# FrancisTheCat/raytracing_c

Measured on AMD Instinct MI355X. Metric: Mray/s, higher is better.
Workload: dtype f32; 1 GPU; helmet.glb 1920x1080, 256 spp, 8 bounces (BASELINE.json configs[2]); partition=single GPU

## Files before the change

### raytracing_c_amd/csrc/rt_dev.hip.h

```cpp
#ifndef RT_DEV_HIP_H
#define RT_DEV_HIP_H

#include <hip/hip_runtime.h>
#include <stdint.h>

#include "rt_device.h"
#include "../../include/rt_math.h"

#ifndef RT_SCALAR_TEX
#define RT_SCALAR_TEX 1
#endif
#ifndef RT_SCALAR_MATS
#define RT_SCALAR_MATS 1
#endif
#ifndef RT_LEAF_PAIRS
#define RT_LEAF_PAIRS 0
#endif

#define RT_BLOCK_WAVES 4
#define RT_BLOCK_THREADS (RT_BLOCK_WAVES * 64)

#define CNT_PATHS 0
#define CNT_RAYS 1
#define CNT_NODES 2
// ... 807 lines not shown
  } else {
    t = normalize_dev(rt_v3_cross(normal, rt_v3_make(1, 0, 0)));
  }
  b = rt_v3_cross(normal, t);

  BrdfIn bi;
  bi.roughness = roughness;
  bi.metalness = metalness;
  bi.base_color = base_color;
  bi.sheen = m2.y;
  bi.sheen_tint = m2.z;
  bi.aniso2 = m2.w * m2.w;

  rt_v3 neg = rt_v3_scale(in.direction, -1.0f);
  rt_v3 in_dir = rt_v3_make(rt_v3_dot(t, neg), rt_v3_dot(b, neg), rt_v3_dot(normal, neg));
  rt_v3 o, rgb;
  float a;
  sample_disney(bi, in_dir, rng, o, rgb, a);

  out_dir = rt_v3_comb3(t, o.x, b, o.y, normal, o.z);
  if (a > 0.0f) {
    tint = rt_v3_make(rgb.x / a, rgb.y / a, rgb.z / a);
  } else {
    terminate = true;
  }
}

template <class PT>
__device__ __forceinline__ void primary_ray(const PT &P, int x, int y, int sample, rt_v3 &o, rt_v3 &d) {
  float inv_width = P.inv_width;
  float inv_height = P.inv_height;
  float aspect = P.aspect;
  float jitter = rt_hash12((float)x * 50.0f + (float)sample, (float)y);
  float uvx = rt_madd(((float)x + jitter - 0.5f) * 2.0f, inv_width, -1.0f);
  float uvy = rt_madd(((float)y + jitter - 0.5f) * 2.0f, inv_height, -1.0f);
  float dx = uvx * aspect, dy = -uvy, dz = -P.focal_length;
  float inv_length = rcp_exact(rt_sqrtf(rt_dot3(dx, dx, dy, dy, dz, dz)));
  float rx = rt_dot3(P.cam[0][0], dx, P.cam[0][1], dy, P.cam[0][2], dz);
  float ry = rt_dot3(P.cam[1][0], dx, P.cam[1][1], dy, P.cam[1][2], dz);
  float rz = rt_dot3(P.cam[2][0], dx, P.cam[2][1], dy, P.cam[2][2], dz);
  o = rt_v3_make(P.cam[0][3], P.cam[1][3], P.cam[2][3]);
  d = rt_v3_make(rx * inv_length, ry * inv_length, rz * inv_length);
}

template <bool SHORT_DIV = false>
__device__ __forceinline__ void ray_setup(Ray3 &r, rt_v3 o, rt_v3 d) {
  r.o = o;
  r.d = d;
  if (SHORT_DIV) {
    r.inv_x = rcp_exact(d.x);
    r.inv_y = rcp_exact(d.y);
    r.inv_z = rcp_exact(d.z);
  } else {
    r.inv_x = 1.0f / d.x;
    r.inv_y = 1.0f / d.y;
    r.inv_z = 1.0f / d.z;
  }
  r.fast = rt_slab_fast(o.x, o.y, o.z, r.inv_x, r.inv_y, r.inv_z, rt_slab_bias(o.x, r.inv_x), rt_slab_bias(o.y, r.inv_y), rt_slab_bias(o.z, r.inv_z));
}

template <class PT>
__device__ __forceinline__ bool shade_hit(const PT &P, const HitRec &hit, rt_v3 &org, rt_v3 &dir,
                                          rt_v3 &tint, rt_v3 &emis, uint32_t &rng, int &bounce,
                                          LaneCounters &cn, rt_v3 &radiance) {
  bool done = false;
  const float *tb = P.tris + (size_t)hit.tri * 28;
  float4 q0 = ld4(tb, 0), q1 = ld4(tb, 1), q2 = ld4(tb, 2), q3 = ld4(tb, 3);
  float4 q4 = ld4(tb, 4), q5 = ld4(tb, 5), q6 = ld4(tb, 6);
  float t1 = hit.u, t2 = hit.v;
  float t0 = 1.0f - t1 - t2;
  rt_v3 point = rt_v3_madd(dir, hit.t, org);
  rt_v3 n_geo = rt_v3_make(q0.x, q0.y, q0.z);
  rt_v3 n_int = rt_v3_make(rt_dot3(q1.x, t0, q2.x, t1, q3.x, t2),
                           rt_dot3(q1.y, t0, q2.y, t1, q3.y, t2),
                           rt_dot3(q1.z, t0, q2.z, t1, q3.z, t2));
  if (rt_v3_dot(n_geo, dir) > 0.0f || rt_v3_dot(n_int, dir) > 0.0f) {
    org = rt_v3_madd(dir, RT_EPS, point);
  } else {
    ShadeIn in;
    in.direction = dir;
    in.normal = normalize_dev(n_int);
    in.tangent = rt_v3_make(q4.x, q4.y, q4.z);
    in.bitangent = rt_v3_make(q5.x, q5.y, q5.z);
    in.uvx = rt_dot3(q1.w, t0, q3.w, t1, q5.w, t2);
    in.uvy = rt_dot3(q2.w, t0, q4.w, t1, q6.x, t2);
    rt_v3 out_dir, s_tint, s_emis;
    bool terminate;
    cn.shades += 1;
    shade(P, as_i(q0.w), in, rng, out_dir, s_tint, s_emis, terminate, cn);
    emis = rt_v3_mul_add(s_emis, tint, emis);
    if (terminate) {
      done = true;
      radiance = emis;
    } else {
      dir = out_dir;
      tint = rt_v3_mul(tint, s_tint);
      float below = (rt_v3_dot(n_geo, out_dir) < 0.0f) ? 1.0f : 0.0f;
      float bias = (0.5f - below) * 2.0f * RT_EPS;
      org = rt_v3_madd(n_geo, bias, point);
    }
  }
  if (!done) {
    bounce += 1;
    if (bounce >= P.max_bounces) {
      done = true;
      radiance = emis;
    }
  }
  return done;
}

#define PH_NEED 0
#define PH_POP  1
#define PH_NODE 2
#define PH_LEAF 3
#define PH_HIT  4
#define PH_MISS 5

#define RT_PARK_FIELDS 18
#define RT_PARK_CAP 128
static_assert(RT_PARK_FIELDS * RT_PARK_CAP == RT_PARK_RECORD_DWORDS, "park slice size (rt_device.h) out of step");
#ifndef RT_PARK_DENSE
#define RT_PARK_DENSE 48
#endif
#ifndef RT_JOIN_CHOICES
#define RT_JOIN_CHOICES 4
#endif
#ifndef RT_PYR_NUM
#define RT_PYR_NUM 3
#define RT_PYR_DEN 4
#define RT_PYR_MIN 8
#endif
#define RT_STEAL_TRIES  16
#ifndef RT_LEAF_TRIP
#define RT_LEAF_TRIP 1
#endif
#ifndef RT_LEAF_CULL_MAX
#define RT_LEAF_CULL_MAX 4
#endif
#ifndef RT_PARK_STOP_PATHS
#define RT_PARK_STOP_PATHS 0
#endif

__device__ __forceinline__ float *lds_at(float4 *smem, int byte_off) {
  asm volatile("" : "+s"(byte_off));
  return reinterpret_cast<float *>(reinterpret_cast<char *>(smem) + byte_off);
}
__device__ __forceinline__ int lane_now() {
  unsigned ones = ~0u;
  asm volatile("" : "+s"(ones));
  return (int)__builtin_amdgcn_mbcnt_hi(ones, __builtin_amdgcn_mbcnt_lo(ones, 0u));
}

__device__ __forceinline__ uint32_t pyramid_cull_mask(const float4 *lds_nodes, const float *pyr, int node) {
  const int lane = lane_now();
  const float *nb = reinterpret_cast<const float *>(lds_nodes + lds_node_f4(node)) + (lane & 7);
  const float *pl = pyr + ((lane >> 3) & 3) * 4;
  const float ox = pyr[16], oy = pyr[17], oz = pyr[18];
  const float mnx = nb[0], mny = nb[8], mnz = nb[16], mxx = nb[24], mxy = nb[32], mxz = nb[40];
  const float nx = pl[0], ny = pl[1], nz = pl[2];
  const bool empty = mnx == 0.0f && mny == 0.0f && mnz == 0.0f && mxx == 0.0f && mxy == 0.0f && mxz == 0.0f;
  const float lox = nx * (mnx - ox), hix = nx * (mxx - ox), loy = ny * (mny - oy), hiy = ny * (mxy - oy);
  const float loz = nz * (mnz - oz), hiz = nz * (mxz - oz);
  const float nearest = fminf(lox, hix) + fminf(loy, hiy) + fminf(loz, hiz);
  const float extent = fmaxf(fabsf(lox), fabsf(hix)) + fmaxf(fabsf(loy), fabsf(hiy)) + fmaxf(fabsf(loz), fabsf(hiz));
  const float coarse = fabsf(nx) * (fabsf(ox) + fmaxf(fabsf(mnx), fabsf(mxx))) + fabsf(ny) * (fabsf(oy) + fmaxf(fabsf(mny), fabsf(mxy))) +
                       fabsf(nz) * (fabsf(oz) + fmaxf(fabsf(mnz), fabsf(mxz)));
  const bool outside = empty || nearest > 1e-3f * extent + 1e-6f * coarse;
  const uint32_t m = (uint32_t)__ballot(outside);
  return (m | (m >> 8) | (m >> 16) | (m >> 24)) & 0xFFu;
}

__device__ __forceinline__ float slab_entry_ordered(const Ray3 &r, const rt_v3 &bs, const char *nbase, int k, int nx, int ny, int nz, float t_max) {
  const char *b = nbase + k * 4;
  const float sx = rt_slab_t_fast(*reinterpret_cast<const float *>(b + nx), r.o.x, r.inv_x, bs.x);
  const float bx = rt_slab_t_fast(*reinterpret_cast<const float *>(b + (96 - nx)), r.o.x, r.inv_x, bs.x);
  const float sy = rt_slab_t_fast(*reinterpret_cast<const float *>(b + 32 + ny), r.o.y, r.inv_y, bs.y);
  const float by = rt_slab_t_fast(*reinterpret_cast<const float *>(b + 32 + (96 - ny)), r.o.y, r.inv_y, bs.y);
  const float sz = rt_slab_t_fast(*reinterpret_cast<const float *>(b + 64 + nz), r.o.z, r.inv_z, bs.z);
  const float bz = rt_slab_t_fast(*reinterpret_cast<const float *>(b + 64 + (96 - nz)), r.o.z, r.inv_z, bs.z);
  const float t_minv = fmax_hw(RT_EPS, fmax_hw(sx, fmax_hw(sy, sz)));
  const float t_maxv = fmin_hw(t_max, fmin_hw(bx, fmin_hw(by, bz)));
  return (t_minv < t_maxv) ? t_minv : RT_INF;
}

__device__ __forceinline__ uint32_t node_enter_few(const Ray3 &r, const float4 *lds_nodes, int node, uint32_t surv,
                                                   float hit_t) {
  const char *nbase = reinterpret_cast<const char *>(lds_nodes + lds_node_f4(node));
  const int nx = (as_i(r.inv_x) >> 31) & 96, ny = (as_i(r.inv_y) >> 31) & 96, nz = (as_i(r.inv_z) >> 31) & 96;
  const rt_v3 bs = slab_bias3(r);
  const int n = (int)__popc(surv);
  const int k0 = (int)__builtin_ctz(surv);
  const int e0 = as_i(slab_entry_ordered(r, bs, nbase, k0, nx, ny, nz, hit_t));
  const uint32_t f0 = 1u - (((uint32_t)e0 + 0x00800000u) >> 31);
  LGM("nfew_ret1");
  if (n == 1) return (uint32_t)k0 | (f0 << 24);
  surv &= surv - 1u;
  const int k1 = (int)__builtin_ctz(surv);
  const int e1 = as_i(slab_entry_ordered(r, bs, nbase, k1, nx, ny, nz, hit_t));
  const uint32_t f1 = 1u - (((uint32_t)e1 + 0x00800000u) >> 31);
  LGM("nfew_two");
  if (n == 2) {
    const bool swap = e1 < e0;
    const uint32_t first = swap ? (uint32_t)k1 : (uint32_t)k0, second = swap ? (uint32_t)k0 : (uint32_t)k1;
    return first | (second << 3) | ((f0 + f1) << 24);
  }
  LGM("nfew_ret2");
  surv &= surv - 1u;
  const int k2 = (int)__builtin_ctz(surv);
  const int e2 = as_i(slab_entry_ordered(r, bs, nbase, k2, nx, ny, nz, hit_t));
  const uint32_t f2 = 1u - (((uint32_t)e2 + 0x00800000u) >> 31);
  int e3 = 0x7F800000, k3 = 0;
  uint32_t f3 = 0;
  LGM("nfew_four_begin");
  if (n == 4) {
    surv &= surv - 1u;
    k3 = (int)__builtin_ctz(surv);
      e3 = as_i(slab_entry_ordered(r, bs, nbase, k3, nx, ny, nz, hit_t));
    f3 = 1u - (((uint32_t)e3 + 0x00800000u) >> 31);
  }
  LGM("nfew_four_end");
  const int e[4] = {e0, e1, e2, e3};
  const int kk[4] = {k0, k1, k2, k3};
  int rank[4] = {0, 1, 2, 3};
#pragma unroll
  for (int j = 0; j < 4; j++) {
#pragma unroll
    for (int k = j + 1; k < 4; k++) {
      int kb = (int)((uint32_t)(e[k] - e[j]) >> 31);
      rank[j] += kb;
      rank[k] -= kb;
    }
  }
  uint32_t w = 0;
#pragma unroll
  for (int j = 0; j < 4; j++) w |= (uint32_t)kk[j] << (3 * rank[j]);
  return w | ((f0 + f1 + f2 + f3) << 24);
}

__device__ __forceinline__ uint32_t pyramid_cull_tris(const float *leaves, const float *pyr, int g) {
  const int lane = lane_now();
  const float *tb = leaves + (size_t)g * 72 + (lane & 7);
  const float *pl = pyr + ((lane >> 3) & 3) * 4;
  const float ox = pyr[16], oy = pyr[17], oz = pyr[18];
  const float nx = pl[0], ny = pl[1], nz = pl[2];
  const float ax = tb[0], e1x = tb[8], e2x = tb[16], ay = tb[24], e1y = tb[32], e2y = tb[40], az = tb[48], e1z = tb[56], e2z = tb[64];
  bool outside = true;
#pragma unroll
  for (int v = 0; v < 3; v++) {
    const float vx = v == 0 ? ax : (v == 1 ? ax + e1x : ax + e2x);
    const float vy = v == 0 ? ay : (v == 1 ? ay + e1y : ay + e2y);
    const float vz = v == 0 ? az : (v == 1 ? az + e1z : az + e2z);
    const float px = nx * (vx - ox), py = ny * (vy - oy), pz = nz * (vz - oz);
    const float val = px + py + pz;
    const float extent = fabsf(px) + fabsf(py) + fabsf(pz);
    const float coarse = fabsf(nx) * (fabsf(ox) + fabsf(vx)) + fabsf(ny) * (fabsf(oy) + fabsf(vy)) + fabsf(nz) * (fabsf(oz) + fabsf(vz));
    outside = outside && (val > 1e-3f * extent + 1e-6f * coarse);
  }
  const uint32_t m = (uint32_t)__ballot(outside);
  return (m | (m >> 8) | (m >> 16) | (m >> 24)) & 0xFFu;
}

template <bool SHORT_DIV>
__device__ __forceinline__ void tri_test_uniform(const Ray3 &r, rt_v3 a, rt_v3 edge1, rt_v3 edge2, int k, float &best, float &bu, float &bv, int &bi) {
  rt_v3 rxe2 = rt_v3_cross(r.d, edge2);
  float det = rt_v3_dot(edge1, rxe2);
  float inv_det = SHORT_DIV ? rcp_leaf(det) : 1.0f / det;
  rt_v3 s = rt_v3_sub(r.o, a);
  rt_v3 sxe1 = rt_v3_cross(s, edge1);
  float u = inv_det * rt_v3_dot(s, rxe2);
  float v = inv_det * rt_v3_dot(r.d, sxe1);
  float t = inv_det * rt_v3_dot(edge2, sxe1);
  bool miss = (u < -RT_EPS) || (u > 1.0f + RT_EPS) || (v < -RT_EPS) || (u + v > 1.0f + RT_EPS) || (t < RT_EPS);
  if (SHORT_DIV) {
    if (!miss && t < best) { best = t; bi = k; bu = u; bv = v; }
  } else {
    float dist = miss ? RT_INF : t;
    dist = (dist > 0.0f) ? dist : RT_INF;
    if (dist < best) { best = dist; bi = k; bu = u; bv = v; }
  }
}
template <bool SHORT_DIV>
__device__ __forceinline__ bool leaf_test_uniform(const RT_KParams &P, const Ray3 &r, int g, uint32_t surv, HitRec &hit) {
  float best = RT_INF, bu = 0.0f, bv = 0.0f;
  int   bi = 0;
  cfloat *lb = as_scalar_ptr(P.leaves) + (size_t)g * 72;
  while (surv) {
    const int k0 = (int)__builtin_ctz(surv);
    surv &= surv - 1u;
#if RT_LEAF_TRIP == 1
    {
      cfloat *t0 = lb + k0;
      tri_test_uniform<SHORT_DIV>(r, rt_v3_make(t0[0], t0[24], t0[48]), rt_v3_make(t0[8], t0[32], t0[56]), rt_v3_make(t0[16], t0[40], t0[64]),
                                  k0, best, bu, bv, bi);
      continue;
    }
#endif
    const bool two = surv != 0u;
    const int k1 = two ? (int)__builtin_ctz(surv) : k0;
    surv &= surv - 1u;
    cfloat *t0 = lb + k0, *t1 = lb + k1;
    const rt_v3 a0 = rt_v3_make(t0[0], t0[24], t0[48]), e10 = rt_v3_make(t0[8], t0[32], t0[56]), e20 = rt_v3_make(t0[16], t0[40], t0[64]);
    const rt_v3 a1 = rt_v3_make(t1[0], t1[24], t1[48]), e11 = rt_v3_make(t1[8], t1[32], t1[56]), e21 = rt_v3_make(t1[16], t1[40], t1[64]);
    tri_test_uniform<SHORT_DIV>(r, a0, e10, e20, k0, best, bu, bv, bi);
    if (two) tri_test_uniform<SHORT_DIV>(r, a1, e11, e21, k1, best, bu, bv, bi);
  }
// ... 288 lines not shown
```

### raytracing_c_amd/csrc/rt_kernels.hip

```cpp

#include "rt_dev.hip.h"


#ifdef RT_LEDGER
#define RT_LEDGER_WAVES 8192
__device__ uint32_t g_ledger[RT_LEDGER_WAVES * RT_LEDGER_ROW];
__global__ void rt_ledger_reduce_kernel(unsigned long long *counters) {
  const int slot = threadIdx.x;
  if (slot >= LG_N || slot >= RT_LEDGER_ROW) return;
  unsigned long long sum = 0ull;
  for (int w = 0; w < RT_LEDGER_WAVES; w++) sum += g_ledger[w * RT_LEDGER_ROW + slot];
  counters[8 + slot] = sum;
}
#endif

typedef const RT_KView __attribute__((address_space(4))) *RT_KViewP;
template <bool VIEWS> struct CamSrc { typedef RT_KArgs type; };
template <> struct CamSrc<true> { typedef RT_KViewP type; };

template <int WAVES, bool LDSN, int MIN_WAVES_PER_SIMD, bool SHORT_DIV, bool VIEWS>
__global__ __launch_bounds__(WAVES * 64, MIN_WAVES_PER_SIMD) void rt_path_kernel_stream(RT_KParams P) {
  extern __shared__ float4 smem[];
  const int lane = threadIdx.x & 63;
  const int wave = threadIdx.x >> 6;
// ... 69 lines not shown
      RT_KArgs A = cold_args();
      const int n_tiles = A->n_tiles;
      const uint32_t *open_groups = A->open_groups, *tile_next = A->tile_next;
      const int n_groups = (n_tiles + 63) >> 6;
      const int g_rounds = (n_groups + 63) >> 6;
      const uint32_t hsh = ((uint32_t)wave_id * 2654435761u + (uint32_t)steal_tries * 40503u) >> 8;
      const int g_start = (int)(hsh % (uint32_t)g_rounds);
      for (int i = 0; i < g_rounds && tile_idx < 0; i++) {
        int r = g_start + i;
        if (r >= g_rounds) r -= g_rounds;
        int g = r * 64 + lane;
        uint32_t n_open = 0;
        if (g < n_groups) n_open = __hip_atomic_load(&open_groups[g], __ATOMIC_RELAXED, __HIP_MEMORY_SCOPE_AGENT);
        unsigned long long gm = __ballot(n_open != 0u);
        while (gm && tile_idx < 0) {
          int nth = (int)((hsh >> 6) % (uint32_t)__popcll(gm));
          unsigned long long m = gm;
          for (int k = 0; k < nth; k++) m &= m - 1ull;
          int gl = (int)__builtin_ctzll(m);
          gm &= ~(1ull << gl);
          int cand = (r * 64 + gl) * 64 + lane;
          uint32_t taken = 0xFFFFFFFFu;
          if (cand < n_tiles) taken = __hip_atomic_load(&tile_next[cand], __ATOMIC_RELAXED, __HIP_MEMORY_SCOPE_AGENT);
          unsigned long long open = __ballot(taken < n_chunks_tile);
          if (open) {
            const int n_open_tiles = (int)__popcll(open);
            int best = 0;
            uint32_t best_taken = 0xFFFFFFFFu;
#pragma unroll
            for (int c = 0; c < RT_JOIN_CHOICES; c++) {
              int nt = (int)(((hsh >> 12) * (uint32_t)(2 * c + 1) + (uint32_t)c * 7u) % (uint32_t)n_open_tiles);
              unsigned long long mm = open;
              for (int k = 0; k < nt; k++) mm &= mm - 1ull;
              const int pk_lane = (int)__builtin_ctzll(mm);
              const uint32_t tk = (uint32_t)__builtin_amdgcn_readlane((int)taken, pk_lane);
              if (tk < best_taken) { best_taken = tk; best = pk_lane; }
            }
            tile_idx = cand - lane + best;
          }
        }
      }
      LGT1(LG_CYC_JOIN);
      if (tile_idx < 0) break;
    }

    int tile_x0, tile_y0;
    RT_KViewP vrec = nullptr;
    {
      RT_KArgs A = cold_args();
      int vt = tile_idx;
      if constexpr (VIEWS) {
        const int tu = __builtin_amdgcn_readfirstlane(tile_idx);
        const uint32_t view = (uint32_t)tu / (uint32_t)A->tiles_per_view;
        vt = tu - (int)view * A->tiles_per_view;
        vrec = (RT_KViewP)A->views + view;
      }
      const int lchunk = vt >> 4, sub = vt & 15;
      const int chunk = A->local_chunks[lchunk];
      const int chunks_x = A->chunks_x;
      tile_x0 = (chunk % chunks_x) * 32 + (sub & 3) * 8;
      tile_y0 = (chunk / chunks_x) * 32 + (sub >> 2) * 8;
      if (tile_x0 >= A->width || tile_y0 >= A->height) {
        if (lane == 0) {
          uint32_t old = atomicMax(&A->tile_next[tile_idx], n_chunks_tile);
          if (old < n_chunks_tile) atomicSub(&A->open_groups[tile_idx >> 6], 1u);
        }
        continue;
      }
    }
    bool tile_root_miss = false;
    if (leaf_level >= 0) {
      RT_KArgs A = cold_args();
      typename CamSrc<VIEWS>::type S;
      if constexpr (VIEWS) S = vrec; else S = A;
      const float m = 0.05f;
      const float ux0 = ((float)tile_x0 - 0.5f - m) * 2.0f * A->inv_width - 1.0f;
      const float ux1 = ((float)tile_x0 + 7.5f + m) * 2.0f * A->inv_width - 1.0f;
      const float uy0 = ((float)tile_y0 - 0.5f - m) * 2.0f * A->inv_height - 1.0f;
      const float uy1 = ((float)tile_y0 + 7.5f + m) * 2.0f * A->inv_height - 1.0f;
      const float asp = A->aspect, fl = S->focal_length;
      rt_v3 c[4];
#pragma unroll
      for (int q = 0; q < 4; q++) {
        float cx = ((q == 1 || q == 2) ? ux1 : ux0) * asp, cy = -((q >= 2) ? uy1 : uy0), cz = -fl;
        c[q] = rt_v3_make(S->cam[0][0] * cx + S->cam[0][1] * cy + S->cam[0][2] * cz,
                          S->cam[1][0] * cx + S->cam[1][1] * cy + S->cam[1][2] * cz,
                          S->cam[2][0] * cx + S->cam[2][1] * cy + S->cam[2][2] * cz);
      }
      const rt_v3 o = rt_v3_make(S->cam[0][3], S->cam[1][3], S->cam[2][3]);
      rt_v3 pn[4];
#pragma unroll
      for (int q = 0; q < 4; q++) {
        rt_v3 n = rt_v3_cross(c[q], c[(q + 1) & 3]);
        if (rt_v3_dot(n, c[(q + 2) & 3]) > 0.0f) n = rt_v3_scale(n, -1.0f);
        pn[q] = n;
      }
      float *pyr = lds_at(smem, pyr_off);
      if (lane == 0) {
#pragma unroll
        for (int q = 0; q < 4; q++) { pyr[q * 4 + 0] = pn[q].x; pyr[q * 4 + 1] = pn[q].y; pyr[q * 4 + 2] = pn[q].z; }
        pyr[16] = o.x; pyr[17] = o.y; pyr[18] = o.z;
      }
      if (lane < 40) reinterpret_cast<uint32_t *>(pyr)[24 + lane] = 0u;
      bool may_hit = false;
      if (lane < 8) {
        const float *nb = P.nodes + lane;
        rt_v3 lo = rt_v3_make(nb[0] - o.x, nb[8] - o.y, nb[16] - o.z);
        rt_v3 hi = rt_v3_make(nb[24] - o.x, nb[32] - o.y, nb[40] - o.z);
        const bool empty = nb[0] == 0.0f && nb[8] == 0.0f && nb[16] == 0.0f && nb[24] == 0.0f && nb[32] == 0.0f && nb[40] == 0.0f;
        bool outside = empty;
#pragma unroll
        for (int q = 0; q < 4; q++) {
          rt_v3 n = pn[q];
          float lox = n.x * lo.x, hix = n.x * hi.x, loy = n.y * lo.y, hiy = n.y * hi.y, loz = n.z * lo.z, hiz = n.z * hi.z;
          float nearest = fminf(lox, hix) + fminf(loy, hiy) + fminf(loz, hiz);
          float extent = fmaxf(fabsf(lox), fabsf(hix)) + fmaxf(fabsf(loy), fabsf(hiy)) + fmaxf(fabsf(loz), fabsf(hiz));
          float coarse = fabsf(n.x) * (fabsf(o.x) + fmaxf(fabsf(nb[0]), fabsf(nb[24]))) + fabsf(n.y) * (fabsf(o.y) + fmaxf(fabsf(nb[8]), fabsf(nb[32]))) +
                         fabsf(n.z) * (fabsf(o.z) + fmaxf(fabsf(nb[16]), fabsf(nb[40])));
          if (nearest > 1e-3f * extent + 1e-6f * coarse) outside = true;
        }
        may_hit = !outside;
      }
      tile_root_miss = __ballot(may_hit) == 0ull;
    }
    const uint32_t rays_before = w_rays;
    LG(LG_TILE_X, 1);
    LGM("tile_end");
    LGT1(LG_CYC_TILE);

    int   phase = PH_NEED;
    int   pix = 0, bounce = 0;
    uint32_t rng = 0;
    Ray3  ray;
    ray_setup(ray, rt_v3_make(0, 0, 0), rt_v3_make(0, 0, 1));
    rt_v3 tint = rt_v3_make(1, 1, 1), emis = rt_v3_make(0, 0, 0);
    int   level = -1, node = 0, child = 0;
    uint32_t cur = 0, dirty = 0, live = 0;
    HitRec hit;
    hit.t = RT_INF; hit.tri = -1; hit.u = 0; hit.v = 0;

    bool tile_open = true;
    int  c_next = 0, c_end = 0, c_x0 = 0, c_y = 0, c_pix0 = 0, c_s0 = 0;
    uint32_t u_cur = 0, u_end = 0, grab = queue_open ? (uint32_t)cold_args()->grab_max : 1u;
    bool took_any = false;
    int  n_parked = 0;
    uint32_t *park = cold_args()->park;

#ifndef RT_NO_SKY_LOOP
    if (tile_root_miss && cold_args()->max_bounces > 0) {
      RT_KArgs A = cold_args();
      typename CamSrc<VIEWS>::type S;
      if constexpr (VIEWS) S = vrec; else S = A;
      const int width = A->width, height = A->height, sample_first = A->sample_first, sample_end = A->sample_end;
      const uint32_t n_sb = (uint32_t)A->n_sample_blocks, gmax = (uint32_t)A->grab_max;
      PrimaryParams PP;
#pragma unroll
      for (int i = 0; i < 3; i++)
#pragma unroll
        for (int j = 0; j < 4; j++) PP.cam[i][j] = S->cam[i][j];
      PP.focal_length = S->focal_length; PP.inv_width = A->inv_width; PP.inv_height = A->inv_height; PP.aspect = A->aspect;
      ShadeParamsLds SP;
      SP.tris = nullptr; SP.mats = nullptr; SP.textures = A->textures; SP.texels = A->texels;
      SP.bg_texture = A->bg_texture; SP.max_bounces = A->max_bounces;
      uint32_t *tile_next = A->tile_next, *open_groups = A->open_groups;
      uint32_t n_sky = 0;
      for (;;) {
        if (c_next >= c_end) {
          if (u_cur + 1u < u_end) {
            u_cur += 1u;
          } else {
            uint32_t u0 = 0;
            if (lane == 0) u0 = atomicAdd(&tile_next[tile_idx], grab);
            u0 = (uint32_t)__builtin_amdgcn_readfirstlane((int)u0);
            if (u0 >= n_chunks_tile) { tile_open = false; break; }
            u_cur = u0;
            u_end = u0 + grab < n_chunks_tile ? u0 + grab : n_chunks_tile;
            if (u_end == n_chunks_tile && lane == 0) atomicSub(&open_groups[tile_idx >> 6], 1u);
            if (t_wave_start) t_last_grab = __builtin_amdgcn_s_memrealtime();
            LG(LG_GRAB_X, 1);
            const uint32_t left = n_chunks_tile - u_end;
            grab = left >= 8u * gmax ? gmax : (left >= 8u && gmax >= 2u ? 2u : 1u);
            took_any = true;
          }
          const uint32_t grp = u_cur >> 2, pair = u_cur & 3u;
          const uint32_t row = grp / n_sb, sb = grp - row * n_sb;
          c_x0 = tile_x0 + (int)pair * 2;
          c_y = tile_y0 + (int)row;
          c_pix0 = (int)row * 8 + (int)pair * 2;
          c_s0 = sample_first + (int)(sb << shift);
          c_next = 0;
          c_end = (c_y < height && c_x0 < width) ? unit_paths : 0;
          continue;
        }
#ifndef RT_SKY_PATHS
#define RT_SKY_PATHS 1
#endif
        LGM("sky_begin");
        LGT0();
        const int avail = c_end - c_next;
        const int take = avail < 64 * RT_SKY_PATHS ? avail : 64 * RT_SKY_PATHS;
        const int l = lane_now();
        bool valid[RT_SKY_PATHS];
        int  pxs[RT_SKY_PATHS];
        rt_v3 dirs[RT_SKY_PATHS];
        bool slow = false;
#pragma unroll
        for (int q = 0; q < RT_SKY_PATHS; q++) {
          const int kq = l + 64 * q;
          const int k = c_next + kq;
          pxs[q] = k >> shift;
          const int sm = c_s0 + (k & ((1 << shift) - 1));
          const int x = c_x0 + pxs[q];
          valid[q] = kq < take && x < width && sm < sample_end;
          rt_v3 o = rt_v3_make(0, 0, 0);
          dirs[q] = rt_v3_make(0, 0, 1);
          Ray3 r;
          if (valid[q]) primary_ray(PP, x, c_y, sm, o, dirs[q]);
          ray_setup<SHORT_DIV>(r, o, dirs[q]);
          slow = slow || (valid[q] && !r.fast);
        }
        if (__ballot(slow) != 0ull) break;
        uint32_t nv = 0;
#pragma unroll
        for (int q = 0; q < RT_SKY_PATHS; q++) {
          if (valid[q]) {
            const rt_v3 bg = background_lookup(SP, dirs[q]);
            const rt_v3 radiance = rt_v3_mul_add(bg, rt_v3_make(1, 1, 1), rt_v3_make(0, 0, 0));
            unsigned long long *ap = reinterpret_cast<unsigned long long *>(lds_at(smem, acc_off) + (c_pix0 + pxs[q]) * 6);
            atomicAdd(ap + 0, accum_quantize_dev(radiance.x));
            atomicAdd(ap + 1, accum_quantize_dev(radiance.y));
            atomicAdd(ap + 2, accum_quantize_dev(radiance.z));
          }
          nv += (uint32_t)__popcll(__ballot(valid[q]));
        }
        w_paths += nv; w_rays += nv; w_nodes += nv; w_bgs += nv;
        n_sky += nv;
        LG(LG_SKY_X, 1); LG(LG_SKY_L, nv);
        c_next += take;
        LGT1(LG_CYC_SKY);
        LGM("sky_end");
      }
      if (n_sky != 0u && lane == 0) atomicAdd(cold_args()->counters + CNT_SKIPPED_ROOT, (unsigned long long)n_sky);
    }
#endif

    for (;;) {
      {
        LGT0();
        LGM("s_begin");
        LG(LG_S_ITER, 1);
        LaneCounters cn;
        cn.rays = cn.nodes = cn.leaves = cn.shades = cn.bgs = cn.textured = cn.paths = 0;
        bool  done = false, start = false, fresh = false;
        rt_v3 radiance = rt_v3_make(0, 0, 0);
        rt_v3 org = ray.o, dir = ray.d;
        RT_KArgs A = cold_args();
        ShadeParamsLds SP;
        SP.tris = A->tris; SP.mats = A->mats; SP.textures = A->textures; SP.texels = A->texels;
        SP.bg_texture = A->bg_texture; SP.max_bounces = A->max_bounces;
#ifdef RT_LEDGER
        { const int n_env = (int)__popcll(__ballot(phase == PH_MISS)); LG(LG_ENV_X, n_env != 0); LG(LG_ENV_L, n_env); }
#endif
        LGM("env_begin");
        if (phase == PH_MISS) {
          cn.bgs = 1;
          rt_v3 bg = background_lookup(SP, dir);
          radiance = rt_v3_mul_add(bg, tint, emis);
          done = true;
        }
        LGM("env_end");
        bool shade_now = true;
        if (park) {
          const unsigned long long mHit = __ballot(phase == PH_HIT);
          const unsigned long long mIdle = __ballot(phase == PH_NEED) | __ballot(phase == PH_MISS);
          const int h = (int)__popcll(mHit), f = (int)__popcll(mIdle);
          const int back = n_parked < f ? n_parked : f;
          uint32_t *pk = park + (size_t)__builtin_amdgcn_readfirstlane(wave_id) * (RT_PARK_FIELDS * RT_PARK_CAP);
          const bool tile_ending = RT_PARK_STOP_PATHS > 0 &&
                                   (int)(n_chunks_tile - u_end) * unit_paths + (int)(u_end - u_cur) * unit_paths <= RT_PARK_STOP_PATHS;
          if (!tile_open || tile_ending || h + back >= RT_PARK_DENSE || n_parked + h > RT_PARK_CAP) {
            if (back > 0) {
              LG(LG_PLOAD_X, 1); LG(LG_PLOAD_L, back);
              LGM("pload_begin");
              if (done) {
                unsigned long long *ap = reinterpret_cast<unsigned long long *>(lds_at(smem, acc_off) + pix * 6);
                atomicAdd(ap + 0, accum_quantize_dev(radiance.x));
                atomicAdd(ap + 1, accum_quantize_dev(radiance.y));
                atomicAdd(ap + 2, accum_quantize_dev(radiance.z));
                phase = PH_NEED;
                done = false;
              }
              const int rank = (int)__builtin_amdgcn_mbcnt_hi((uint32_t)(mIdle >> 32), __builtin_amdgcn_mbcnt_lo((uint32_t)mIdle, 0u));
              if (phase == PH_NEED && rank < back) {
                const uint32_t *q = pk + (n_parked - 1 - rank);
                uint32_t v[RT_PARK_FIELDS];
                __builtin_amdgcn_fence(__ATOMIC_ACQUIRE, "wavefront");
#pragma unroll
                for (int i = 0; i < RT_PARK_FIELDS; i++)
                  v[i] = __hip_atomic_load(q + i * RT_PARK_CAP, __ATOMIC_RELAXED, __HIP_MEMORY_SCOPE_AGENT);
                hit.t = as_f((int)v[0]); hit.tri = (int)v[1]; hit.u = as_f((int)v[2]); hit.v = as_f((int)v[3]);
                org = rt_v3_make(as_f((int)v[4]), as_f((int)v[5]), as_f((int)v[6]));
                dir = rt_v3_make(as_f((int)v[7]), as_f((int)v[8]), as_f((int)v[9]));
                tint = rt_v3_make(as_f((int)v[10]), as_f((int)v[11]), as_f((int)v[12]));
                emis = rt_v3_make(as_f((int)v[13]), as_f((int)v[14]), as_f((int)v[15]));
                rng = v[16]; pix = (int)(v[17] & 63u); bounce = (int)(v[17] >> 6);
                phase = PH_HIT;
              }
              n_parked -= back;
              LGM("pload_end");
            }
          } else if (h > 0) {
            LG(LG_PSTORE_X, 1); LG(LG_PSTORE_L, h);
            LGM("pstore_begin");
            shade_now = false;
            const int rank = (int)__builtin_amdgcn_mbcnt_hi((uint32_t)(mHit >> 32), __builtin_amdgcn_mbcnt_lo((uint32_t)mHit, 0u));
            if (phase == PH_HIT) {
              uint32_t *q = pk + (n_parked + rank);
              const uint32_t v[RT_PARK_FIELDS] = {(uint32_t)as_i(hit.t), (uint32_t)hit.tri, (uint32_t)as_i(hit.u), (uint32_t)as_i(hit.v),
                                                  (uint32_t)as_i(org.x), (uint32_t)as_i(org.y), (uint32_t)as_i(org.z),
                                                  (uint32_t)as_i(dir.x), (uint32_t)as_i(dir.y), (uint32_t)as_i(dir.z),
                                                  (uint32_t)as_i(tint.x), (uint32_t)as_i(tint.y), (uint32_t)as_i(tint.z),
                                                  (uint32_t)as_i(emis.x), (uint32_t)as_i(emis.y), (uint32_t)as_i(emis.z),
                                                  rng, (uint32_t)pix | ((uint32_t)bounce << 6)};
#pragma unroll
              for (int i = 0; i < RT_PARK_FIELDS; i++) q[i * RT_PARK_CAP] = v[i];
              __builtin_amdgcn_fence(__ATOMIC_RELEASE, "wavefront");
              phase = PH_NEED;
            }
            n_parked += h;
            LGM("pstore_end");
          }
        }
#ifdef RT_LEDGER
        { const int n_sh = (int)__popcll(__ballot(phase == PH_HIT && shade_now)); LG(LG_SHADE_X, n_sh != 0); LG(LG_SHADE_L, n_sh); }
#endif
        LGM("shade_begin");
        if (phase == PH_HIT && shade_now) {
          done = shade_hit(SP, hit, org, dir, tint, emis, rng, bounce, cn, radiance);
          start = !done;
        }
        LGM("shade_end");
#ifdef RT_LEDGER
        { const int n_acc = (int)__popcll(__ballot(done)); LG(LG_ACCUM_X, n_acc != 0); LG(LG_ACCUM_L, n_acc); }
#endif
        LGM("accum_begin");
        if (done) {
          unsigned long long *ap = reinterpret_cast<unsigned long long *>(lds_at(smem, acc_off) + pix * 6);
          atomicAdd(ap + 0, accum_quantize_dev(radiance.x));
          atomicAdd(ap + 1, accum_quantize_dev(radiance.y));
          atomicAdd(ap + 2, accum_quantize_dev(radiance.z));
          phase = PH_NEED;
        }
        LGM("accum_end");
        w_shades += (uint32_t)__popcll(__ballot(cn.shades != 0));
        w_tex += (uint32_t)__popcll(__ballot(cn.textured != 0));
        w_bgs += (uint32_t)__popcll(__ballot(cn.bgs != 0));

        if (tile_open) {
          unsigned long long need = __ballot(phase == PH_NEED);
          bool got = false;
          int  gx = 0, gy = 0, gs = 0, gp = 0;
          const int width = A->width, sample_end = A->sample_end;
          LGM("regen_begin");
          while (need) {
            LG(LG_REGEN_X, 1);
            if (c_next >= c_end) {
              if (u_cur + 1u < u_end) {
                u_cur += 1u;
              } else {
                uint32_t u0 = 0;
                if (lane == 0) u0 = atomicAdd(&A->tile_next[tile_idx], grab);
                u0 = (uint32_t)__builtin_amdgcn_readfirstlane((int)u0);
                if (u0 >= n_chunks_tile) {
                  tile_open = false;
                  LGD0((int)__popcll(__ballot(phase != PH_NEED || got)) + n_parked);
                  break;
                }
                u_cur = u0;
                u_end = u0 + grab < n_chunks_tile ? u0 + grab : n_chunks_tile;
                if (u_end == n_chunks_tile && lane == 0) atomicSub(&A->open_groups[tile_idx >> 6], 1u);
                LG(LG_GRAB_X, 1);
                if (t_wave_start) t_last_grab = __builtin_amdgcn_s_memrealtime();
                const uint32_t left = n_chunks_tile - u_end;
                const uint32_t gmax = (uint32_t)A->grab_max;
                grab = left >= 8u * gmax ? gmax : (left >= 8u && gmax >= 2u ? 2u : 1u);
                took_any = true;
              }
              const uint32_t grp = u_cur >> 2, pair = u_cur & 3u;
              const uint32_t n_sb = (uint32_t)A->n_sample_blocks;
              const uint32_t row = grp / n_sb, sb = grp - row * n_sb;
              c_x0 = tile_x0 + (int)pair * 2;
              c_y = tile_y0 + (int)row;
              c_pix0 = (int)row * 8 + (int)pair * 2;
              c_s0 = A->sample_first + (int)(sb << shift);
              c_next = 0;
              c_end = (c_y < A->height && c_x0 < width) ? unit_paths : 0;
              continue;
            }
            const int n_need = (int)__popcll(need);
            const int avail = c_end - c_next;
            const int take = n_need < avail ? n_need : avail;
            const int rank = (int)__builtin_amdgcn_mbcnt_hi((uint32_t)(need >> 32), __builtin_amdgcn_mbcnt_lo((uint32_t)need, 0u));
            bool valid = false;
            if (phase == PH_NEED && !got && rank < take) {
              int k = c_next + rank;
              int px = k >> shift;
              int sm = c_s0 + (k & ((1 << shift) - 1));
              int x = c_x0 + px;
              if (x < width && sm < sample_end) {
                valid = true;
                if (SP.max_bounces > 0) { got = true; gx = x; gy = c_y; gs = sm; gp = c_pix0 + px; }
              }
            }
            w_paths += (uint32_t)__popcll(__ballot(valid));
            c_next += take;
            need = __ballot(phase == PH_NEED && !got);
          }
          LGM("regen_end");
#ifdef RT_LEDGER
          { const int n_pr = (int)__popcll(__ballot(got)); LG(LG_PRIM_X, n_pr != 0); LG(LG_PRIM_L, n_pr); LG(LG_REGEN_L, n_pr); }
#endif
          LGM("prim_begin");
          if (got) {
            typename CamSrc<VIEWS>::type S;
            if constexpr (VIEWS) S = vrec; else S = A;
            pix = gp;
            bounce = 0;
            rng = rt_path_seed(S->seed, (uint32_t)(gx + gy * width), (uint32_t)gs);
            PrimaryParams PP;
#pragma unroll
            for (int i = 0; i < 3; i++)
#pragma unroll
              for (int j = 0; j < 4; j++) PP.cam[i][j] = S->cam[i][j];
            PP.focal_length = S->focal_length; PP.inv_width = A->inv_width; PP.inv_height = A->inv_height; PP.aspect = A->aspect;
            primary_ray(PP, gx, gy, gs, org, dir);
            tint = rt_v3_make(1, 1, 1);
            emis = rt_v3_make(0, 0, 0);
            start = true;
            fresh = true;
          }
          LGM("prim_end");
        }
        bool skip_root = false;
#ifdef RT_LEDGER
        { const int n_st = (int)__popcll(__ballot(start)); LG(LG_START_X, n_st != 0); LG(LG_START_L, n_st); }
#endif
        LGM("start_begin");
        if (start) {
          ray_setup<SHORT_DIV>(ray, org, dir);
          hit.t = RT_INF; hit.tri = -1; hit.u = 0; hit.v = 0;
          dirty = 0;
          live = 0;
          cur = 0;
          level = -1;
          node = 0;
          child = (leaf_level >= 0) ? 0 : P.last_row_offset;
          phase = (leaf_level >= 0) ? PH_NODE : PH_LEAF;
          skip_root = fresh && tile_root_miss && ray.fast;
          if (skip_root) phase = PH_MISS;
        }
        LGM("start_end");
        w_rays += (uint32_t)__popcll(__ballot(start));
        {
          const uint32_t n_skip = (uint32_t)__popcll(__ballot(skip_root));
          w_nodes += n_skip;
          if (n_skip != 0u && lane == 0) atomicAdd(cold_args()->counters + CNT_SKIPPED_ROOT, (unsigned long long)n_skip);
        }
        LGM("s_end");
        LGT1(LG_CYC_S);
      }

      const int n_trav0 = (int)__popcll(__ballot(phase == PH_NODE || phase == PH_LEAF));
      if (n_trav0 == 0) {
        if (__any(phase == PH_MISS)) continue;
        if (n_parked > 0 || __any(phase == PH_HIT)) continue;
        if (!tile_open) break;
        continue;
      }

      traversal_blocks<LDSN, SHORT_DIV, true>(P, smem, lds_nodes, perm, lane, n_lds, pyr_nodes, pyr_off, leaf_level,
                                              tile_open ? thresh : drain_thresh, n_trav0, ray, bounce == 0, phase, level, node,
                                              child, cur, dirty, live, hit, w_nodes, w_leaves LG_ARG);
    }

    LGD1();
    LGM("flush_begin");
    if (took_any) {
      LGT0();
      LG(LG_FLUSH_X, 1);
      int x = tile_x0 + (lane & 7), y = tile_y0 + (lane >> 3);
      unsigned long long r = acc[lane * 3 + 0], g = acc[lane * 3 + 1], b = acc[lane * 3 + 2];
      acc[lane * 3 + 0] = 0ull;
      acc[lane * 3 + 1] = 0ull;
      acc[lane * 3 + 2] = 0ull;
      RT_KArgs A = cold_args();
      const int width = A->width;
      if (x < width && y < A->height && (r | g | b) != 0ull) {
        unsigned long long *base = A->accum;
        if constexpr (VIEWS) base += (size_t)(vrec - (RT_KViewP)A->views) * (size_t)A->pixels_per_view * 3;
        unsigned long long *dst = base + ((size_t)y * width + x) * 3;
        atomicAdd(dst + 0, r);
        atomicAdd(dst + 1, g);
        atomicAdd(dst + 2, b);
      }
      uint32_t *tile_cost = A->tile_cost;
      if (tile_cost && lane == 0) atomicAdd(&tile_cost[tile_idx], w_rays - rays_before);
      steal_tries = 0;
      n_tiles_done += 1;
      LGT1(LG_CYC_FLUSH);
    }
  }
  RT_KArgs A = cold_args();
  unsigned long long *wave_times = A->wave_times, *counters = A->counters;
  if (wave_times && lane == 0 && wave_id < 65536) {
    wave_times[wave_id * 3 + 0] = t_wave_start;
    wave_times[wave_id * 3 + 1] = __builtin_amdgcn_s_memrealtime();
    wave_times[wave_id * 3 + 2] = ((t_last_grab - t_wave_start) << 16) | (n_tiles_done & 0xFFFFu);
  }

  if (lane == 0) {
    atomicAdd(counters + CNT_PATHS, (unsigned long long)w_paths);
    atomicAdd(counters + CNT_RAYS, (unsigned long long)w_rays);
    atomicAdd(counters + CNT_NODES, (unsigned long long)w_nodes);
    atomicAdd(counters + CNT_LEAVES, (unsigned long long)w_leaves);
    atomicAdd(counters + CNT_SHADES, (unsigned long long)w_shades);
    atomicAdd(counters + CNT_BG, (unsigned long long)w_bgs);
    atomicAdd(counters + CNT_TEXTURED, (unsigned long long)w_tex);
#ifdef RT_LEDGER
    LG(LG_CYC_WAVE, (uint32_t)((__builtin_amdgcn_s_memtime() - lg_wave_t0) >> 4));
#endif
  }
}

__global__ void rt_resolve_kernel(int width, int height, int samples, int chunks_x, const int32_t *local_chunks,
                                  int n_local_chunks, const unsigned long long *accum,
                                  uint8_t *tiles, uint8_t *image, float *linear) {
  int idx = blockIdx.x * blockDim.x + threadIdx.x;
  if (idx >= n_local_chunks * 1024) return;
  int lchunk = idx >> 10, p = idx & 1023;
  int chunk = local_chunks[lchunk];
  int x = (chunk % chunks_x) * 32 + (p & 31);
  int y = (chunk / chunks_x) * 32 + (p >> 5);
  uint8_t rgb[3] = {0, 0, 0};
  if (x < width && y < height) {
    size_t pix = (size_t)y * width + x;
#pragma unroll
    for (int c = 0; c < 3; c++) {
      float lin = rt_accum_resolve(accum[pix * 3 + c], (uint32_t)samples);
      if (linear) linear[pix * 3 + c] = lin;
      rgb[c] = rt_encode_u8(lin);
      if (image) image[pix * 3 + c] = rgb[c];
    }
  }
  if (tiles) {
    tiles[(size_t)idx * 3 + 0] = rgb[0];
    tiles[(size_t)idx * 3 + 1] = rgb[1];
    tiles[(size_t)idx * 3 + 2] = rgb[2];
  }
}

__global__ void rt_untile_kernel(int width, int height, int chunks_x, int n_chunks, const int32_t *owner_slot,
                                 const uint8_t *all_tiles, uint8_t *image) {
  int idx = blockIdx.x * blockDim.x + threadIdx.x;
  if (idx >= n_chunks * 1024) return;
// ... 325 lines not shown
```

Before: 21730 Mray/s.

## Remap sky-tile work units to pixel-per-lane and accumulate in registers

```diff
diff --git a/raytracing_c_amd/csrc/rt_dev.hip.h b/raytracing_c_amd/csrc/rt_dev.hip.h
--- a/raytracing_c_amd/csrc/rt_dev.hip.h
+++ b/raytracing_c_amd/csrc/rt_dev.hip.h
@@ -983,6 +983,12 @@
   return (int)__builtin_amdgcn_mbcnt_hi(ones, __builtin_amdgcn_mbcnt_lo(ones, 0u));
 }
 
+__device__ __forceinline__ void sky_unit_decode(uint32_t u, int unit_paths, int sample_first, int &pix0, int &s0) {
+  const uint32_t j0 = u * (uint32_t)unit_paths;
+  pix0 = (int)(j0 & 63u);
+  s0 = sample_first + (int)(j0 >> 6);
+}
+
 __device__ __forceinline__ uint32_t pyramid_cull_mask(const float4 *lds_nodes, const float *pyr, int node) {
   const int lane = lane_now();
   const float *nb = reinterpret_cast<const float *>(lds_nodes + lds_node_f4(node)) + (lane & 7);
diff --git a/raytracing_c_amd/csrc/rt_kernels.hip b/raytracing_c_amd/csrc/rt_kernels.hip
--- a/raytracing_c_amd/csrc/rt_kernels.hip
+++ b/raytracing_c_amd/csrc/rt_kernels.hip
@@ -245,7 +245,7 @@
       typename CamSrc<VIEWS>::type S;
       if constexpr (VIEWS) S = vrec; else S = A;
       const int width = A->width, height = A->height, sample_first = A->sample_first, sample_end = A->sample_end;
-      const uint32_t n_sb = (uint32_t)A->n_sample_blocks, gmax = (uint32_t)A->grab_max;
+      const uint32_t gmax = (uint32_t)A->grab_max;
       PrimaryParams PP;
 #pragma unroll
       for (int i = 0; i < 3; i++)
@@ -257,6 +257,10 @@
       SP.bg_texture = A->bg_texture; SP.max_bounces = A->max_bounces;
       uint32_t *tile_next = A->tile_next, *open_groups = A->open_groups;
       uint32_t n_sky = 0;
+      const int l = lane_now();
+      const int lx = tile_x0 + (l & 7), ly = tile_y0 + (l >> 3);
+      const bool in_image = lx < width && ly < height;
+      unsigned long long sum_r = 0ull, sum_g = 0ull, sum_b = 0ull;
       for (;;) {
         if (c_next >= c_end) {
           if (u_cur + 1u < u_end) {
@@ -275,63 +279,43 @@
             grab = left >= 8u * gmax ? gmax : (left >= 8u && gmax >= 2u ? 2u : 1u);
             took_any = true;
           }
-          const uint32_t grp = u_cur >> 2, pair = u_cur & 3u;
-          const uint32_t row = grp / n_sb, sb = grp - row * n_sb;
-          c_x0 = tile_x0 + (int)pair * 2;
-          c_y = tile_y0 + (int)row;
-          c_pix0 = (int)row * 8 + (int)pair * 2;
-          c_s0 = sample_first + (int)(sb << shift);
+          sky_unit_decode(u_cur, unit_paths, sample_first, c_pix0, c_s0);
           c_next = 0;
-          c_end = (c_y < height && c_x0 < width) ? unit_paths : 0;
+          c_end = unit_paths;
           continue;
         }
-#ifndef RT_SKY_PATHS
-#define RT_SKY_PATHS 1
-#endif
         LGM("sky_begin");
         LGT0();
         const int avail = c_end - c_next;
-        const int take = avail < 64 * RT_SKY_PATHS ? avail : 64 * RT_SKY_PATHS;
-        const int l = lane_now();
-        bool valid[RT_SKY_PATHS];
-        int  pxs[RT_SKY_PATHS];
-        rt_v3 dirs[RT_SKY_PATHS];
-        bool slow = false;
-#pragma unroll
-        for (int q = 0; q < RT_SKY_PATHS; q++) {
-          const int kq = l + 64 * q;
-          const int k = c_next + kq;
-          pxs[q] = k >> shift;
-          const int sm = c_s0 + (k & ((1 << shift) - 1));
-          const int x = c_x0 + pxs[q];
-          valid[q] = kq < take && x < width && sm < sample_end;
-          rt_v3 o = rt_v3_make(0, 0, 0);
-          dirs[q] = rt_v3_make(0, 0, 1);
-          Ray3 r;
-          if (valid[q]) primary_ray(PP, x, c_y, sm, o, dirs[q]);
-          ray_setup<SHORT_DIV>(r, o, dirs[q]);
-          slow = slow || (valid[q] && !r.fast);
-        }
-        if (__ballot(slow) != 0ull) break;
-        uint32_t nv = 0;
-#pragma unroll
-        for (int q = 0; q < RT_SKY_PATHS; q++) {
-          if (valid[q]) {
-            const rt_v3 bg = background_lookup(SP, dirs[q]);
-            const rt_v3 radiance = rt_v3_mul_add(bg, rt_v3_make(1, 1, 1), rt_v3_make(0, 0, 0));
-            unsigned long long *ap = reinterpret_cast<unsigned long long *>(lds_at(smem, acc_off) + (c_pix0 + pxs[q]) * 6);
-            atomicAdd(ap + 0, accum_quantize_dev(radiance.x));
-            atomicAdd(ap + 1, accum_quantize_dev(radiance.y));
-            atomicAdd(ap + 2, accum_quantize_dev(radiance.z));
-          }
-          nv += (uint32_t)__popcll(__ballot(valid[q]));
-        }
+        const int take = avail < 64 ? avail : 64;
+        const int sm = c_s0 + (c_next >> 6);
+        if (sm >= sample_end) { c_next += take; continue; }
+        const bool valid = in_image && (uint32_t)(l - c_pix0) < (uint32_t)take;
+        rt_v3 o = rt_v3_make(0, 0, 0), dir = rt_v3_make(0, 0, 1);
+        Ray3 r;
+        if (valid) primary_ray(PP, lx, ly, sm, o, dir);
+        ray_setup<SHORT_DIV>(r, o, dir);
+        if (__ballot(valid && !r.fast) != 0ull) break;
+        if (valid) {
+          const rt_v3 bg = background_lookup(SP, dir);
+          const rt_v3 radiance = rt_v3_mul_add(bg, rt_v3_make(1, 1, 1), rt_v3_make(0, 0, 0));
+          sum_r += accum_quantize_dev(radiance.x);
+          sum_g += accum_quantize_dev(radiance.y);
+          sum_b += accum_quantize_dev(radiance.z);
+        }
+        const uint32_t nv = (uint32_t)__popcll(__ballot(valid));
         w_paths += nv; w_rays += nv; w_nodes += nv; w_bgs += nv;
         n_sky += nv;
         LG(LG_SKY_X, 1); LG(LG_SKY_L, nv);
         c_next += take;
         LGT1(LG_CYC_SKY);
         LGM("sky_end");
+      }
+      {
+        unsigned long long *ap = reinterpret_cast<unsigned long long *>(lds_at(smem, acc_off) + l * 6);
+        ap[0] += sum_r;
+        ap[1] += sum_g;
+        ap[2] += sum_b;
       }
       if (n_sky != 0u && lane == 0) atomicAdd(cold_args()->counters + CNT_SKIPPED_ROOT, (unsigned long long)n_sky);
     }
@@ -479,6 +463,12 @@
                 grab = left >= 8u * gmax ? gmax : (left >= 8u && gmax >= 2u ? 2u : 1u);
                 took_any = true;
               }
+              if (tile_root_miss) {
+                sky_unit_decode(u_cur, unit_paths, A->sample_first, c_pix0, c_s0);
+                c_next = 0;
+                c_end = unit_paths;
+                continue;
+              }
               const uint32_t grp = u_cur >> 2, pair = u_cur & 3u;
               const uint32_t n_sb = (uint32_t)A->n_sample_blocks;
               const uint32_t row = grp / n_sb, sb = grp - row * n_sb;
@@ -499,10 +489,18 @@
               int k = c_next + rank;
               int px = k >> shift;
               int sm = c_s0 + (k & ((1 << shift) - 1));
-              int x = c_x0 + px;
-              if (x < width && sm < sample_end) {
+              int x = c_x0 + px, y = c_y, p = c_pix0 + px;
+              bool inside = x < width;
+              if (tile_root_miss) {
+                p = c_pix0 + (k & 63);
+                sm = c_s0 + (k >> 6);
+                x = tile_x0 + (p & 7);
+                y = tile_y0 + (p >> 3);
+                inside = x < width && y < A->height;
+              }
+              if (inside && sm < sample_end) {
                 valid = true;
-                if (SP.max_bounces > 0) { got = true; gx = x; gy = c_y; gs = sm; gp = c_pix0 + px; }
+                if (SP.max_bounces > 0) { got = true; gx = x; gy = y; gs = sm; gp = p; }
               }
             }
             w_paths += (uint32_t)__popcll(__ballot(valid));
```

After: 21770 Mray/s, median of 6. About the same (+0.2%).
